# craabreu/EmDee.jl

Hardware: AMD Instinct MI355X
Metric: md_steps_per_sec (higher is better)
Workload: dtype f64

## Files before the change

emdee.jl_amd/csrc/brick.hpp:

```cpp
#pragma once

#include "kernels.hpp"

namespace emdee {

enum BrickMode { BRICK_FORCE = 1, BRICK_STATS = 2, BRICK_STEP = 3 };

#define EMDEE_PLAIN_LOOP _Pragma("clang loop unroll(disable) vectorize(disable) interleave(disable)")

constexpr int EPL = 8;
constexpr int brick_prefetch_blocks(int G, int THREADS) { return (EPL * G) >= 128 ? 1 : ((G == 4 && THREADS >= 1024) ? 5 : 2); }
constexpr int brick_min_stride(int G, int THREADS) { return (brick_prefetch_blocks(G, THREADS) + 1) * EPL * G; }

template <int BX_, int BY_, int BZ_>
struct BrickShape {
    static constexpr int BX = BX_, BY = BY_, BZ = BZ_;
    static constexpr int TX = BX + 2, TY = BY + 2, TZ = BZ + 2;
    static constexpr int NTC = TX * TY * TZ;
    static constexpr int NOC = BX * BY * BZ;
};

struct BrickGrid {
    int nb[3];
    int nbricks;
    int per_xcd;
    int ib_lo[3], ib_n[3];
    int ib_count, ib_per_xcd;
    int bb_z, bb_y, bb_count, bb_per_xcd;
};

__host__ __device__ __forceinline__ int outside_interval(int k, int lo, int n) { return k < lo ? k : k + n; }

template <typename real>
__device__ __forceinline__ void tile_load(const Rec<real> *tile, const float *tile_te, int s, real &x, real &y, real &z,
                                          real &hs, real &te);
template <>
__device__ __forceinline__ void tile_load<double>(const Rec<double> *tile, const float *, int s, double &x, double &y,
                                                  double &z, double &hs, double &te) {
    Rec<double> r = tile[s];
    x = r.x; y = r.y; z = r.z; hs = (double)r.hs; te = (double)r.te;
}
template <>
__device__ __forceinline__ void tile_load<float>(const Rec<float> *tile, const float *tile_te, int s, float &x, float &y,
                                                 float &z, float &hs, float &te) {
    Rec<float> r = tile[s];
// ... 306 lines not shown

template <typename real, class Shape, int THREADS>
__global__ __launch_bounds__(THREADS) void k_brick_tables(BrickArgs<real> a) {
    extern __shared__ __attribute__((aligned(16))) unsigned char s_dyn[];
    BrickTables<Shape, THREADS> T;
    T.carve(s_dyn);
    const int lb = (blockIdx.x % NXCD) * a.bg.per_xcd + blockIdx.x / NXCD;
    if (lb >= a.bg.nbricks) return;
    int bxi = 0, byi = 0, bzi = 0, tile_n = 0, n_own = 0;
    brick_setup<real, Shape, THREADS, true>(a, T, bxi, byi, bzi, tile_n, n_own);
    constexpr int ROW = BrickTables<Shape, THREADS>::row_ints(), IMG = BrickTables<Shape, THREADS>::image_ints();
    int *row = a.btab + (size_t)(bxi + a.bg.nb[0] * (byi + a.bg.nb[1] * bzi)) * ROW;
    for (int i = threadIdx.x; i < IMG; i += THREADS) row[i] = T.off[i];
    if (threadIdx.x == 0) { row[IMG] = tile_n; row[IMG + 1] = n_own; }
    if (a.stats != nullptr) {
        int span3 = 0;
        if (threadIdx.x < Shape::NTC && threadIdx.x % Shape::TX + 3 <= Shape::TX) span3 = T.off[threadIdx.x + 3] - T.off[threadIdx.x];
#pragma unroll
        for (int off = 1; off < WAVE; off <<= 1) span3 = max(span3, __shfl_xor(span3, off));
        int *maxima = reinterpret_cast<int *>(a.stats);
        if ((threadIdx.x & (WAVE - 1)) == 0 && span3 > __hip_atomic_load(&maxima[2], __ATOMIC_RELAXED, __HIP_MEMORY_SCOPE_AGENT)) atomicMax(&maxima[2], span3);
        if (threadIdx.x == 0) {
            if (tile_n - 1 > __hip_atomic_load(&maxima[0], __ATOMIC_RELAXED, __HIP_MEMORY_SCOPE_AGENT)) atomicMax(&maxima[0], tile_n - 1);
            if (n_own > __hip_atomic_load(&maxima[1], __ATOMIC_RELAXED, __HIP_MEMORY_SCOPE_AGENT)) atomicMax(&maxima[1], n_own);
        }
    }
}

constexpr int OWN_REGS = 2;

constexpr int BUILD2_FIELD = 16;

template <typename real, class Shape, int THREADS, int G, int ALG = 1, int GL = G>
__global__ __launch_bounds__(THREADS, (THREADS <= 768 ? 6 : 4)) void k_brick_build(BrickArgs<real> a) {
    constexpr int BX = Shape::BX, BY = Shape::BY, TX = Shape::TX, TY = Shape::TY;
    constexpr int NGROUPS = (THREADS / WAVE) * (WAVE / G);
    extern __shared__ __attribute__((aligned(16))) unsigned char s_dyn[];
    float4 *tile = reinterpret_cast<float4 *>(s_dyn);
    BrickTables<Shape, THREADS> T;
    T.carve(s_dyn + (size_t)a.tile_cap * 16);
    int bxi, byi, bzi, tile_n, n_own;
    if (!brick_setup<real, Shape, THREADS>(a, T, bxi, byi, bzi, tile_n, n_own)) return;
    const int tid = threadIdx.x, lane = tid & (WAVE - 1);
    constexpr bool SUBOK = ALG == 3 || ALG == 5 || ALG == 13 || ALG == 15;
    const int NSUB = (SUBOK && a.nsub == 4 && a.bsub != nullptr) ? 4 : 1;
    unsigned *rtab = reinterpret_cast<unsigned *>(s_dyn + (size_t)a.tile_cap * 16 + BrickTables<Shape, THREADS>::bytes(a.own_cap) +
                                                  (size_t)NGROUPS * a.stride * 2);
    int *s_sub = reinterpret_cast<int *>(s_dyn + (size_t)a.tile_cap * 16 + BrickTables<Shape, THREADS>::bytes(a.own_cap));
    auto rt_get = [](const unsigned *rt, int r) { const unsigned v = rt[r]; return make_int2((int)(v & 0xffffu), (int)(v >> 16)); };
    if (NSUB > 1) {
        const int *bs = a.bsub + (size_t)(bxi + a.bg.nb[0] * (byi + a.bg.nb[1] * bzi)) * Shape::NTC;
        for (int i = tid; i < Shape::NTC; i += THREADS) s_sub[i] = bs[i];
        __syncthreads();
    }
    auto own_sub = [&](int oc, int ti) {
        if (NSUB == 1) return 0;
        const int tc = (oc % BX + 1) + TX * (((oc / BX) % BY + 1) + TY * (oc / (BX * BY) + 1));
        const int kk = ti - T.off[tc], pk = s_sub[tc];
        return (kk >= (pk & 1023) ? 1 : 0) + (kk >= ((pk >> 10) & 1023) ? 1 : 0) + (kk >= ((pk >> 20) & 1023) ? 1 : 0);
    };

    real org[3] = {0, 0, 0};
    if (sizeof(real) == 8) {
        org[0] = a.g.lo[0] + (real)(bxi * BX) * (a.g.len[0] / (real)a.g.M[0]);
        org[1] = a.g.lo[1] + (real)(byi * BY) * (a.g.len[1] / (real)a.g.M[1]);
        org[2] = a.g.lo[2] + (real)(bzi * Shape::BZ) * (a.g.len[2] / (real)a.g.M[2]);
    }
// ... 65 lines not shown
    unsigned short *rowbuf = reinterpret_cast<unsigned short *>(s_dyn + (size_t)a.tile_cap * 16 +
                                                                BrickTables<Shape, THREADS>::bytes(a.own_cap)) +
                             (size_t)gid * a.stride;
    static_assert(G <= 32, "build kernel: groups of at most 32 lanes");
    const unsigned gshift = (unsigned)(lane & 31 & ~(G - 1));
    const unsigned gmask = G == 32 ? 0xffffffffu : ((1u << G) - 1u);
    const unsigned ltmask = (1u << gl) - 1u;
    const bool upper = lane >= 32;
    const unsigned ustride = (unsigned)a.stride;
    const uint4 fill = make_uint4(0, 0, 0, 0);
    auto in_range_q = [&](const float4 &qi, const float4 &qj, int p, int c, int tcr) -> bool {
        const float dx = qi.x - qj.x, dy2 = qi.y - qj.y, dz2 = qi.z - qj.z;
        const float d2 = dx * dx + dy2 * dy2 + dz2 * dz2;
        bool pass = d2 < lo2;
        if (sizeof(real) == 8 && __builtin_expect(!pass && d2 <= hi2, 0)) {
            const int tc = tcr + (c >= T.off[tcr + 1] ? 1 : 0) + (c >= T.off[tcr + 2] ? 1 : 0);
            const int sh = T.shift[tc];
            const Rec<real> ri = a.rec[p], rj = a.rec[__float_as_int(qj.w)];
            const real ex = ri.x - (rj.x + (real)((sh & 3) - 1) * a.g.len[0]);
            const real ey = ri.y - (rj.y + (real)(((sh >> 2) & 3) - 1) * a.g.len[1]);
            const real ez = ri.z - (rj.z + (real)(((sh >> 4) & 3) - 1) * a.g.len[2]);
            pass = ex * ex + ey * ey + ez * ez < a.rlist2;
        }
        return pass;
    };
    auto in_range = [&](const float4 &qi, int p, int c, int tcr) -> bool { return in_range_q(qi, tile[c], p, c, tcr); };
    if constexpr (ALG % 10 == 3 || ALG % 10 == 5) {
        static_assert(G == 4 || G == 8 || G == 16, "two-phase build: 4, 8 or 16 lanes per atom");
        constexpr int FIELD = ALG % 10 == 3 ? BUILD2_FIELD : 32, PER = 32 / FIELD;
        constexpr int NROWS = 9, NWORDS = (NROWS + PER - 1) / PER;
        constexpr bool BAND = sizeof(real) == 8;
        constexpr int UNR = 2;
        float nrl2 = -rl2, nmargin_v = BAND ? -a.margin : 0.f, margin_v = a.margin;
        asm volatile("" : "+v"(nrl2), "+v"(nmargin_v), "+v"(margin_v));
        constexpr bool STRIDED = ALG >= 10;
        constexpr bool OPP = PER == 2;
        auto row_word = [](int r) constexpr { return OPP ? (r <= 4 ? r : 8 - r) : r / PER; };
        auto row_half = [](int r) constexpr { return OPP ? (r > 4 ? 1 : 0) : r % PER; };
        constexpr int LOG2G = G == 4 ? 2 : (G == 8 ? 3 : 4), KSTEP = STRIDED ? G : 1;
        const int wave_first = __builtin_amdgcn_readfirstlane((tid / WAVE) * (WAVE / G));
        for (int ob = 0; ob < n_own; ob += NGROUPS) {
            if (ob + wave_first >= n_own) break;
            const int o = ob + gid;
            const bool have = o < n_own;
            const int2 info = have ? T.oinfo[o] : make_int2(0, 0);
            const int ti = info.y & 0xffff, p = info.x, oc = info.y >> 20;
            const bool act = have && ((info.y >> 16) & 1) != 0;
            const float4 qi = tile[ti];
            unsigned short *row = a.nbr + (size_t)p * a.stride;
            for (int c = gl * EPL; c < a.stride; c += G * EPL) *reinterpret_cast<uint4 *>(rowbuf + c) = fill;
            unsigned word[NWORDS];
            int cbase[NROWS];
            const unsigned *rt = rtab + (act ? oc * NSUB + ((info.y >> 17) & 3) : Shape::NOC * NSUB) * 9;
            int2 rv_next = rt_get(rt, 0);
            int trips_of[NROWS];
            auto chunk_of = [&](int r) { return (int)((unsigned)(rt_get(rt, r).y + G - 1) / (unsigned)G); };
            int cv = chunk_of(min(gl, NROWS - 1));
            int cw = G == 4 ? chunk_of(4 + gl) : 0;
            int c8 = chunk_of(NROWS - 1);
            auto ror4 = [](int v) { return max(v, __builtin_amdgcn_update_dpp(0, v, 0x124 , 0xf, 0xf, true)); };
            auto ror8 = [](int v) { return max(v, __builtin_amdgcn_update_dpp(0, v, 0x128 , 0xf, 0xf, true)); };
            if constexpr (G == 4) { cv = ror4(cv); cw = ror4(cw); c8 = ror4(c8); }
            if constexpr (G <= 8) {
                cv = ror8(cv); c8 = ror8(c8);
                if constexpr (G == 4) cw = ror8(cw);
            }
            auto rows_max = [](int v) {
// ... 92 lines not shown
                    if constexpr (STRIDED) {
                        const int d = ti - c0;
                        if ((d & (G - 1)) == gl) bits &= ~(1u << (d >> LOG2G));
                    } else {
                        const int ks = ti - cb;
                        if (ks >= 0 && ks < lim) bits &= ~(1u << ks);
                    }
                }
                if (row_half(r)) word[row_word(r)] |= bits << (row_half(r) * FIELD);
                else word[row_word(r)] = bits;
            }
            int mine = 0;
#pragma unroll
            for (int w = 0; w < NWORDS; w++) mine += __popc(word[w]);
            int incl = mine;
            {
                int t = __builtin_amdgcn_update_dpp(0, incl, DPP_ROW_SHR1, 0xf, 0xf, true);
                incl += gl >= 1 ? t : 0;
                t = __builtin_amdgcn_update_dpp(0, incl, DPP_ROW_SHR2, 0xf, 0xf, true);
                incl += gl >= 2 ? t : 0;
                if (G >= 8) {
                    t = __builtin_amdgcn_update_dpp(0, incl, DPP_ROW_SHR4, 0xf, 0xf, true);
                    incl += gl >= 4 ? t : 0;
                }
                if (G == 16) {
                    t = __builtin_amdgcn_update_dpp(0, incl, DPP_ROW_SHR8, 0xf, 0xf, true);
                    incl += gl >= 8 ? t : 0;
                }
            }
            unsigned short *ep = rowbuf + (unsigned)(incl - mine), *const ep_last = rowbuf + (ustride - 1u);
#pragma unroll
            for (int w = 0; w < NWORDS; w++) {
                unsigned W = word[w];
                int cA = cbase[OPP ? w : PER * w] << a.idx_shift,
                    cB = (OPP ? (w < 4 ? cbase[8 - w] : 0) : ((PER == 2 && 2 * w + 1 < NROWS) ? cbase[2 * w + 1] : 0)) << a.idx_shift;
                asm volatile("" : "+v"(cA), "+v"(cB));
                const int kshift = a.idx_shift + (STRIDED ? LOG2G : 0);
                while (W) {
                    const int k = __ffs((int)W) - 1;
                    W &= W - 1;
                    asm volatile("" : "+v"(W));
                    *(ep < ep_last ? ep : ep_last) = (unsigned short)((k << kshift) + ((PER == 2 && k >= FIELD) ? cB : cA));
                    ep++;
                }
            }
            if (have && EMDEE_BOUND(BS_BUILD_ROW, p, a.n)) {
                constexpr int BLKL = EPL * GL;
                EMDEE_PLAIN_LOOP
                for (int c = gl * EPL; c < a.stride; c += G * EPL) {
                    const unsigned short *src = rowbuf + (c / BLKL) * BLKL + (c % BLKL) / EPL;
                    uint4 q;
                    q.x = (unsigned)src[0 * GL] | ((unsigned)src[1 * GL] << 16);
                    q.y = (unsigned)src[2 * GL] | ((unsigned)src[3 * GL] << 16);
                    q.z = (unsigned)src[4 * GL] | ((unsigned)src[5 * GL] << 16);
                    q.w = (unsigned)src[6 * GL] | ((unsigned)src[7 * GL] << 16);
                    *reinterpret_cast<uint4 *>(row + c) = q;
                }
                if (gl == G - 1) {
                    a.cnt[p] = act ? (int)min((unsigned)incl, ustride) : 0;
                    if ((unsigned)incl > ustride) atomicMax(&a.flags[0], incl);
                }
            }
        }
        return;
    }
    for (int ob = 0; ob < n_own; ob += NGROUPS) {
        const int o = ob + gid;
        const bool have = o < n_own;
// ... 10 lines not shown
#pragma unroll 1
            for (int dy = -1; dy <= 1; dy++) {
                const int tcr = ox + TX * ((oy + 1 + dy) + TY * (oz + 1 + dz));
                const int c0 = T.off[tcr];
                const int span = act ? T.off[tcr + 3] - c0 : 0;
                const int wspan = wave_group_max<G>(span);
                for (int cb = 0; cb < wspan; cb += G) {
                    const int c = c0 + cb + gl;
                    bool pass = false;
                    if (cb + gl < span && c != ti) pass = in_range(qi, p, c, tcr);
                    const unsigned long long mask = __ballot(pass);
                    const unsigned half = upper ? (unsigned)(mask >> 32) : (unsigned)mask;
                    const unsigned bits = (half >> gshift) & gmask;
                    if (pass) {
                        const unsigned e = count + __popc(bits & ltmask);
                        if (e < ustride && EMDEE_BOUND(BS_BUILD_ROWBUF, row_position<GL>(e), ustride)) rowbuf[row_position<GL>(e)] = (unsigned short)(c << a.idx_shift);
                    }
                    count += __popc(bits);
                }
            }
        }
        if (have && EMDEE_BOUND(BS_BUILD_ROW, p, a.n)) {
            for (int c = gl * EPL; c < a.stride; c += G * EPL)
                *reinterpret_cast<uint4 *>(row + c) = *reinterpret_cast<const uint4 *>(rowbuf + c);
            if (gl == 0) {
                a.cnt[p] = act ? (int)min(count, ustride) : 0;
                if (count > ustride) atomicMax(&a.flags[0], (int)count);
            }
        }
    }
}

template <typename real, class Shape, int THREADS, int G, int MODE, int BITMASK_Q, bool UNI = false>
__global__ __launch_bounds__(THREADS) void k_brick(BrickArgs<real> a) {
    constexpr int BITMASK = BITMASK_Q & ~EMDEE_CHARGED;
    constexpr bool CHG = (BITMASK_Q & EMDEE_CHARGED) != 0;
    static_assert(!CHG || (!UNI && MODE == BRICK_FORCE), "charged instances: general-species force launches only");
    constexpr int NGROUPS = (THREADS / WAVE) * (WAVE / G);
    constexpr int BLK = EPL * G;

    extern __shared__ __attribute__((aligned(16))) unsigned char s_dyn[];
    constexpr bool SOA = UNI && MODE != BRICK_STATS;
    constexpr bool FAST = SOA && BITMASK == EMDEE_FORCES;
    Rec<real> *tile = reinterpret_cast<Rec<real> *>(s_dyn);
    real *plane = reinterpret_cast<real *>(s_dyn);
    constexpr int PITCH = soa_pitch<real>();
    const size_t tile_bytes = SOA ? (((size_t)3 * PITCH * sizeof(real) + 15) & ~(size_t)15) : (size_t)a.tile_cap * sizeof(Rec<real>);
    const size_t te_bytes = (sizeof(real) == 4 && !SOA) ? (((size_t)a.tile_cap * 4 + 15) & ~(size_t)15) : 0;
    float *tile_te = reinterpret_cast<float *>(s_dyn + tile_bytes);
    const size_t q_bytes = CHG ? brick_charge_lds_bytes<real>(a.tile_cap) : 0;
    real *tile_q = reinterpret_cast<real *>(s_dyn + tile_bytes + te_bytes);
    BrickTables<Shape, THREADS> T;
    T.carve(s_dyn + tile_bytes + te_bytes + q_bytes);
    if (MODE == BRICK_STEP && a.guard != nullptr && *a.guard != 0) {
        if (threadIdx.x == 0) *a.trigger = 1;
        return;
    }
    int bxi, byi, bzi, tile_n, n_own;
    if (!brick_setup<real, Shape, THREADS>(a, T, bxi, byi, bzi, tile_n, n_own)) return;
    const int tid = threadIdx.x, lane = tid & (WAVE - 1);
    int own_p[OWN_REGS], own_ti[OWN_REGS], own_m[OWN_REGS];
#pragma unroll
    for (int k = 0; k < OWN_REGS; k++) {
        const int o = tid + k * THREADS;
        own_p[k] = own_ti[k] = own_m[k] = 0;
        if (o < n_own) {
            brick_locate(T, o, own_ti[k], own_p[k]);
// ... 131 lines not shown
                    if (ina | inb) {
                        const f32x2 inv = {fast_rcp(r2.x), fast_rcp(r2.y)};
                        const f32x2 sg2 = {(float)a.uni_sigma2, (float)a.uni_sigma2}, e4v = {(float)a.uni_e4, (float)a.uni_e4};
                        if (BITMASK == EMDEE_FORCES) {
                            f32x2 wr2 = lj_force_over_r2_2(r2, inv, mdl, sg2, e4v);
                            wr2 = f32x2{ina ? wr2.x : 0.f, inb ? wr2.y : 0.f};
                            pfx += wr2 * dx; pfy += wr2 * dy; pfz += wr2 * dz;
                        } else {
                            f32x2 E, W;
                            lj_interaction_pair2(r2, inv, mdl, sg2, e4v, E, W);
                            E = f32x2{ina ? E.x : 0.f, inb ? E.y : 0.f};
                            W = f32x2{ina ? W.x : 0.f, inb ? W.y : 0.f};
                            if (BITMASK & EMDEE_FORCES) {
                                const f32x2 wr2 = W * inv;
                                pfx += wr2 * dx; pfy += wr2 * dy; pfz += wr2 * dz;
                            }
                            if (BITMASK & EMDEE_ENERGIES) pe += E;
                            if (BITMASK & EMDEE_VIRIALS) pw += W;
                            if (BITMASK & EMDEE_TENSOR) {
                                const f32x2 wr2 = W * inv, hx = wr2 * dx, hy = wr2 * dy, hz = wr2 * dz;
                                ptxx += hx * dx; ptyy += hy * dy; ptzz += hz * dz;
                                ptxy += hx * dy; ptxz += hx * dz; ptyz += hy * dz;
                            }
                        }
                    }
                }
            }
        };
        auto block = [&](const uint4 &q, int b0) {
            if constexpr (PACKED) {
                block2(q, b0);
                return;
            }
            constexpr bool AHEAD = SOA && BITMASK == EMDEE_FORCES;
            real xn = 0, yn = 0, zn = 0;
            if (AHEAD) {
                const unsigned char *pn = plane_b + pick16(q, 0);
                xn = *reinterpret_cast<const real *>(pn); yn = *reinterpret_cast<const real *>(pn + PLANE_BYTES);
                zn = *reinterpret_cast<const real *>(pn + 2 * PLANE_BYTES);
            }
#pragma unroll
            for (int t = 0; t < EPL; t++) {
                if (b0 + t * G >= wm) break;
                {
                    const int sj = SOA ? pick16(q, t) : (pick16(q, t) >> a.idx_shift);
                    real xj, yj, zj, hs_j, te_j;
                    if (AHEAD) {
                        xj = xn; yj = yn; zj = zn;
                        if (t + 1 < EPL) {
                            const unsigned char *pj = plane_b + pick16(q, t + 1);
                            xn = *reinterpret_cast<const real *>(pj); yn = *reinterpret_cast<const real *>(pj + PLANE_BYTES);
                            zn = *reinterpret_cast<const real *>(pj + 2 * PLANE_BYTES);
                        }
                        hs_j = te_j = 0;
                    } else if (SOA) {
                        const unsigned char *pj = plane_b + sj;
                        xj = *reinterpret_cast<const real *>(pj);
                        yj = *reinterpret_cast<const real *>(pj + PLANE_BYTES);
                        zj = *reinterpret_cast<const real *>(pj + 2 * PLANE_BYTES);
                        hs_j = te_j = 0;
                    } else tile_load<real>(tile, tile_te, sj, xj, yj, zj, hs_j, te_j);
                    real dx = xi - xj, dy = yi - yj, dz = zi - zj;
                    if (REL && MODE == BRICK_FORCE && !SOA) {
                        if (refmath) {
                            dx = a.g.len[0] * (dx - rint(dx)); dy = a.g.len[1] * (dy - rint(dy)); dz = a.g.len[2] * (dz - rint(dz));
                        }
                    }
                    const real r2 = dx * dx + dy * dy + dz * dz;
                    if (MODE == BRICK_STATS) {
                        st_inside += (b0 + t * G + gl < m && r2 < a.model.rc2) ? 1ull : 0ull;
                    } else if (FAST) {
                        if (r2 < uni.rc2) {
                            const real wr2 = lj_force_over_r2_uni(r2, uni);
                            fx += wr2 * dx; fy += wr2 * dy; fz += wr2 * dz;
                        }
                    } else if (r2 < a.model.rc2) {
                        const real inv_r2 = fast_rcp(r2);
                        if (BITMASK == EMDEE_FORCES) {
                            real wr2;
                            if (UNI) {
                                wr2 = lj_force_over_r2(r2, inv_r2, mdl, a.uni_sigma2, a.uni_e4);
                            } else {
                                const real sg = hs_i + hs_j;
                                wr2 = lj_force_over_r2(r2, inv_r2, mdl, sg * sg, te_i * te_j);
                            }
                            if (CHG) wr2 += rf_force_over_r2(r2, inv_r2, q_i * tile_q[sj], a.chg);
                            fx += wr2 * dx; fy += wr2 * dy; fz += wr2 * dz;
                        } else {
                            real E, W;
                            if (UNI) {
                                lj_interaction_pair(r2, inv_r2, mdl, a.uni_sigma2, a.uni_e4, E, W);
                            } else {
                                lj_interaction(r2, inv_r2, mdl, hs_i, te_i, hs_j, te_j, E, W);
                            }
                            if (CHG) {
                                real Ec, Wc;
                                rf_pair(r2, q_i * tile_q[sj], a.chg, Ec, Wc);
                                E += Ec; W += Wc;
                            }
                            if (BITMASK & EMDEE_FORCES) {
                                const real wr2 = W * inv_r2;
// ... 216 lines not shown
```

emdee.jl_amd/csrc/nbsys.hpp:

```cpp
#pragma once
#include <cstdio>

#include <algorithm>
#include <cmath>
#include <cstdlib>
#include <type_traits>

#include "brick.hpp"
#include "kernels.hpp"
#include "typed.hpp"

namespace emdee {

static inline void refuse_experiment_switches() {
    static const char *const gone[] = {"EMDEE_DEBUG_RC2_SCALE", "EMDEE_TBUILD", "EMDEE_BUILD4", "EMDEE_BUILD_ALG", "EMDEE_BUILD_CHUNKED",
        "EMDEE_BUILD_STRIDED", "EMDEE_NO_BRICK_TABLES", "EMDEE_NO_PREMUL", "EMDEE_BUILD_NEARFAR", "EMDEE_NEAR_DELTA", "EMDEE_FAR_SKIP",
        "EMDEE_PLAN_MAXIMA", "EMDEE_PLAN_SYNC", "EMDEE_STRIDE", "EMDEE_BRICK_VARIANT"};
    for (const char *name : gone)
        EMDEE_REQUIRE(std::getenv(name) == nullptr, EMDEE_ERR_INVALID,
                      "%s is an experiment switch that has been retired with the laboratory (make EXPERIMENTS=1 no longer "
                      "exists): the variant it selected is not built; its measurement is recorded in DESIGN.md, "
                      "\"Product and laboratory\"", name);
}

enum TimerId { T_FORCE = 0, T_KICK_DRIFT = 1, T_REBUILD = 2, T_KICK = 3, T_STEP = 4, T_STEP_BOUNDARY = 5, T_HALO = 6, T_COUNT = 7 };
enum PathId { PATH_BRICK = 0, PATH_DIRECT = 1 };

struct Scanner {
    DevBuf<int> scratch;
    void run(int *data, size_t n, hipStream_t s) {
        if (n == 0) return;
        if (n <= (size_t)SCAN_BLOCK_MAX) {
            hipLaunchKernelGGL(k_scan_block, dim3(1), dim3(1024), 0, s, data, (int)n);
            return;
        }
        size_t total = 0;
        for (size_t m = n; m > 1;) {
            m = (m + SCAN_TILE - 1) / SCAN_TILE;
            total += m;
            if (m == 1) break;
        }
        scratch.ensure(total + 1);
        level(data, n, scratch.ptr, s);
    }

  private:
    void level(int *data, size_t n, int *sums, hipStream_t s) {
        size_t tiles = (n + SCAN_TILE - 1) / SCAN_TILE;
        hipLaunchKernelGGL(k_scan_tiles, dim3((unsigned)tiles), dim3(SCAN_THREADS), 0, s, data, data, n,
                           tiles > 1 ? sums : nullptr);
        if (tiles > 1) {
            level(sums, tiles, sums + tiles, s);
            hipLaunchKernelGGL(k_scan_add, dim3(blocks_for(n, 256)), dim3(256), 0, s, data, n, sums);
        }
    }
};

constexpr size_t LDS_LIMIT = 160 * 1024;

template <int V>
struct BrickVariant;
template <> struct BrickVariant<0> { using Shape = BrickShape<4, 2, 2>; static constexpr int THREADS = 512, G = 4, GB = 8; };
template <> struct BrickVariant<7> { using Shape = BrickShape<4, 2, 2>; static constexpr int THREADS = 1024, G = 4, GB = 8; };
template <> struct BrickVariant<8> { using Shape = BrickShape<4, 2, 2>; static constexpr int THREADS = 1024, G = 8, GB = G; };
template <> struct BrickVariant<9> { using Shape = BrickShape<2, 2, 2>; static constexpr int THREADS = 512, G = 4, GB = 8; };

template <class F>
static inline void with_brick_variant(int v, F &&f) {
    switch (v) {
        case 7: f(BrickVariant<7>{}); break;
        case 8: f(BrickVariant<8>{}); break;
        case 9: f(BrickVariant<9>{}); break;
        default: f(BrickVariant<0>{}); break;
    }
}

template <typename K>
static inline void allow_big_lds(K kernel, size_t bytes) {
    if (bytes > 48 * 1024)
        EMDEE_HIP_CHECK(hipFuncSetAttribute(reinterpret_cast<const void *>(kernel),
                                            hipFuncAttributeMaxDynamicSharedMemorySize, (int)bytes));
}

struct PairTables {
    DevBuf<int> x_start, x_idx;
    DevBuf<int> p_start, p_idx;
    std::vector<int32_t> excl, p14;
    double scale14 = 1.0;
    int rows = 0;
// ... 252 lines not shown
    DevBuf<int> perm, perm2, inv_perm, cell_of, cell_sorted, cell_sorted2, order, count, fill, nbr, cnt, flags, img, img2;
    DevBuf<int2> tmp2;
    DevBuf<long long> tag, tag2;
    bool use_tags = false;
    size_t cap_hint = 0;
    size_t capacity = 0;
    bool has_ghosts = false;
    int id_space = 0;
    bool id_gaps = false;
    DevBuf<int> cmap;
    bool cmap_valid = false;
    SpeciesTable species{1, {0, 0, 0, 0}};
    int nt = 1;
    int nsub = 1;
    bool subbins_enabled = std::getenv("EMDEE_NO_SUBBINS") == nullptr;
    int tsub = 1;
    bool typed_subbins_enabled = std::getenv("EMDEE_TYPED_SUBBINS") == nullptr || std::atoi(std::getenv("EMDEE_TYPED_SUBBINS")) != 0;
    int digits() const { return nt > 1 ? nt * tsub : nsub; }
    DevBuf<int> bsub;
    bool typed_enabled = std::getenv("EMDEE_NO_TYPED") == nullptr;
    DevBuf<int> cstart;
    DevBuf<unsigned long long> species_tab;
    DevBuf<unsigned short> nbr16;
    DevBuf<int> btab;
    bool btab_valid = false;
    DevBuf<double> partial, sums;
    DevBuf<unsigned long long> stats;
    Scanner scanner;

    NbSystem() {
        refuse_experiment_switches();
        if (const char *e = std::getenv("EMDEE_PATH")) path = (std::string(e) == "direct") ? PATH_DIRECT : PATH_BRICK;
        if (const char *e = std::getenv("EMDEE_RUN_AHEAD")) run_ahead = std::max(1, std::min(RUN_AHEAD, std::atoi(e)));
    }

    hipStream_t stream() const { return ctx->stream; }
    AtomView<real> view() const { return AtomView<real>{rec.ptr, te.ptr, rel_grid(rel_now, cell_sorted.ptr)}; }

    bool rel_now = false;
    double rel_lo[3] = {0, 0, 0}, rel_cw[3] = {1, 1, 1};
    int rel_M[3] = {1, 1, 1};
    bool rel_wanted() const {
        return sizeof(real) == 4 && with_vel && !with_mass && !use_tags && !has_ghosts && path == PATH_BRICK &&
               std::getenv("EMDEE_F32_ABS") == nullptr;
    }
    RelGrid rel_grid(bool on, const int *cells) const {
        RelGrid r{};
        for (int d = 0; d < 3; d++) { r.lo[d] = rel_lo[d]; r.cw[d] = rel_cw[d]; r.M[d] = rel_M[d]; }
        r.on = on ? 1 : 0;
        r.cell = cells;
        return r;
    }
    RelGrid rel_grid_next(bool on, const int *cells) const {
        RelGrid r{};
        for (int d = 0; d < 3; d++) { r.lo[d] = (double)grid.lo[d]; r.cw[d] = (double)grid.len[d] / (double)grid.M[d]; r.M[d] = grid.M[d]; }
        r.on = on ? 1 : 0;
        r.cell = cells;
        return r;
    }
    void rel_commit(bool on) {
        rel_now = on;
        for (int d = 0; d < 3; d++) { rel_lo[d] = (double)grid.lo[d]; rel_cw[d] = (double)grid.len[d] / (double)grid.M[d]; rel_M[d] = grid.M[d]; }
    }

    struct Timed {
        NbSystem *s;
// ... 316 lines not shown
            const size_t lds = typed_force_lds_bytes<real, typename V::Shape, V::THREADS>(own_cap);
            allow_big_lds(kernel, lds);
            const int phase = (MODE == BRICK_FORCE || MODE == BRICK_STEP) ? force_phase : 0;
            const int blocks = (phase == 1 ? bgrid.ib_per_xcd : phase == 2 ? bgrid.bb_per_xcd : bgrid.per_xcd) * NXCD;
            if (blocks == 0) return;
            hipLaunchKernelGGL(kernel, dim3(blocks), dim3(V::THREADS), lds, stream(), brick_args(phase));
        }
    }

    template <class V>
    static constexpr bool charged_variant() { return std::is_same<V, BrickVariant<0>>::value || std::is_same<V, BrickVariant<8>>::value; }
    template <class V, int MODE, int BM>
    void launch_brick_kernel() {
        if (typed_active) { launch_typed_kernel<V, MODE, BM>(); return; }
        if constexpr (MODE == BRICK_FORCE && (BM == 1 || BM == 7 || BM == TENSOR_PASS)) {
            if (has_charges()) {
                if constexpr (charged_variant<V>()) launch_brick_kernel_impl<V, MODE, BM | EMDEE_CHARGED, false>();
                else EMDEE_REQUIRE(false, EMDEE_ERR_STATE, "charged engine on brick variant %d", variant);
                return;
            }
        }
        if constexpr (std::is_same<V, BrickVariant<0>>::value && (MODE == BRICK_STEP || (MODE == BRICK_FORCE && (BM == 1 || BM == 7 || BM == TENSOR_PASS)))) {
            if (uniform_atoms && tile_cap <= SOA_SLOTS && idx_shift == PLANE_SHIFT && !(MODE == BRICK_FORCE && sizeof(real) == 4 && refmath && ref_pos != nullptr)) {
                launch_brick_kernel_impl<V, MODE, BM, true>();
                return;
            }
        }
        launch_brick_kernel_impl<V, MODE, BM, false>();
    }

    template <class V, int MODE, int BM, bool UNI>
    void launch_brick_kernel_impl() {
        auto kernel = k_brick<real, typename V::Shape, V::THREADS, V::G, MODE, BM, UNI>;
        const size_t lds = (UNI && MODE != BRICK_STATS) ? brick_force_lds_bytes_soa<real, typename V::Shape, V::THREADS>(own_cap)
                                                        : lds_bytes;
        allow_big_lds(kernel, lds);
        const int phase = (MODE == BRICK_FORCE || MODE == BRICK_STEP) ? force_phase : 0;
        const int blocks = (phase == 1 ? bgrid.ib_per_xcd : phase == 2 ? bgrid.bb_per_xcd : bgrid.per_xcd) * NXCD;
        if (blocks == 0) return;
        hipLaunchKernelGGL(kernel, dim3(blocks), dim3(V::THREADS), lds, stream(), brick_args(phase));
    }

    template <class V>
    void launch_brick_force(int bitmask) {
        if constexpr (std::is_same<V, BrickVariant<0>>::value) {
            switch (bitmask) {
                case 1: launch_brick_kernel<V, BRICK_FORCE, 1>(); return;
                case 2: launch_brick_kernel<V, BRICK_FORCE, 2>(); return;
                case 3: launch_brick_kernel<V, BRICK_FORCE, 3>(); return;
                case 4: launch_brick_kernel<V, BRICK_FORCE, 4>(); return;
                case 5: launch_brick_kernel<V, BRICK_FORCE, 5>(); return;
                case 6: launch_brick_kernel<V, BRICK_FORCE, 6>(); return;
                case TENSOR_PASS: launch_brick_kernel<V, BRICK_FORCE, TENSOR_PASS>(); return;
                default: launch_brick_kernel<V, BRICK_FORCE, 7>(); return;
            }
        }
        if (bitmask == 1) launch_brick_kernel<V, BRICK_FORCE, 1>();
        else if (bitmask == TENSOR_PASS) launch_brick_kernel<V, BRICK_FORCE, TENSOR_PASS>();
        else launch_brick_kernel<V, BRICK_FORCE, 7>();
    }

    void plan_geometry() {
        with_brick_variant(variant, [&](auto v) {
            using V = decltype(v);
            using S = typename V::Shape;
            bgrid.nb[0] = (grid.M[0] + S::BX - 1) / S::BX;
            bgrid.nb[1] = (grid.M[1] + S::BY - 1) / S::BY;
            bgrid.nb[2] = (grid.M[2] + S::BZ - 1) / S::BZ;
            bgrid.nbricks = bgrid.nb[0] * bgrid.nb[1] * bgrid.nb[2];
            bgrid.per_xcd = (bgrid.nbricks + NXCD - 1) / NXCD;
            const int B[3] = {S::BX, S::BY, S::BZ};
            bgrid.ib_count = 1;
            for (int d = 0; d < 3; d++) {
                int lo_b = 0, n_b = bgrid.nb[d];
                if (!grid.per[d]) {
                    lo_b = 1;
                    int hi_b = 1;
                    while (hi_b < bgrid.nb[d] && (hi_b + 1) * B[d] < grid.M[d] - 1) hi_b++;
                    n_b = std::max(0, hi_b - lo_b);
                }
                bgrid.ib_lo[d] = lo_b; bgrid.ib_n[d] = n_b;
                bgrid.ib_count *= n_b;
            }
            bgrid.ib_per_xcd = (bgrid.ib_count + NXCD - 1) / NXCD;
            bgrid.bb_z = (bgrid.nb[2] - bgrid.ib_n[2]) * bgrid.nb[0] * bgrid.nb[1];
            bgrid.bb_y = bgrid.ib_n[2] * (bgrid.nb[1] - bgrid.ib_n[1]) * bgrid.nb[0];
            bgrid.bb_count = bgrid.nbricks - bgrid.ib_count;
            bgrid.bb_per_xcd = (bgrid.bb_count + NXCD - 1) / NXCD;
            row_block = EPL * V::G;
        });
    }
    void launch_tile_max(bool with_build_words = false) {
        with_brick_variant(variant, [&](auto v) {
            using S = typename decltype(v)::Shape;
            if (with_build_words) Zeros().add(flags.ptr, 9).run(stream());
            else Zeros().add(flags.ptr + 6, 3).run(stream());
            hipLaunchKernelGGL((k_brick_tile_max<S>), dim3(blocks_for(bgrid.nbricks, 256)), dim3(256), 0, stream(), bgrid,
                               grid.M[0], grid.M[1], grid.M[2], grid.per[0], grid.per[1], grid.per[2], start(),
                               flags.ptr + 6);
        });
    }
    static int with_headroom(int v) { return (v + v / 32 + 8 + 15) / 16 * 16; }
    bool plan_sizes(int max_tile, int max_own, int max_span3) {
        bool ok = true;
        with_brick_variant(variant, [&](auto v) {
            using V = decltype(v);
            using S = typename V::Shape;
            tile_cap = std::max(64, with_headroom(max_tile + 1));
            if (max_tile + 1 <= SOA_SLOTS) tile_cap = std::min(tile_cap, SOA_SLOTS);
            own_cap = std::max(64, with_headroom(max_own));
            {
                const int exact = std::max(64, (max_tile + 1 + 15) / 16 * 16), st = stride > 0 ? stride : 128;
                constexpr size_t USABLE = 150000;
                auto per_cu = [&](int tc) {
                    const size_t b = brick_build_lds_bytes<S, V::THREADS>(tc, own_cap, st, V::GB, nsub),
                                 f = brick_force_lds_bytes<real, S, V::THREADS>(tc, own_cap, has_charges());
                    return (int)(USABLE / std::max<size_t>(b, 1)) * 16 + (int)(USABLE / std::max<size_t>(f, 1));
                };
                while (tile_cap > exact && per_cu(tile_cap) < per_cu(exact)) tile_cap -= 16;
            }
            plan_span3 = max_span3 + max_span3 / 16 + 2;
            if (std::getenv("EMDEE_DEBUG_PLAN"))
                std::fprintf(stderr, "emdee plan: bricks %d x %d x %d, tile_cap %d (max %d), own_cap %d (max %d), max 3-cell span %d, x sub-bins %d K %d\n", bgrid.nb[0],
                             bgrid.nb[1], bgrid.nb[2], tile_cap, max_tile, own_cap, max_own, max_span3, nsub, sub_k());
            build_alg = (!field16_blocked && (V::GB == 8 || V::GB == 16) && plan_span3 <= BUILD2_FIELD * V::GB) ? 3 : 1;
            if (build_alg == 1 && (V::GB == 8 || V::GB == 16) && plan_span3 <= 32 * V::GB) build_alg = 5;
            if (build_alg == 1) plan_span3 = 1 << 30;
            else plan_span3 = (build_alg == 5 ? 32 : BUILD2_FIELD) * V::GB;
            lds_bytes = brick_force_lds_bytes<real, S, V::THREADS>(tile_cap, own_cap, has_charges());
            ok = lds_bytes <= LDS_LIMIT && tile_cap < 65536;
            build_margin = 0.f;
            if (sizeof(real) == 8) {
                double cmax = 0.0;
                const int B[3] = {S::BX, S::BY, S::BZ};
                for (int d = 0; d < 3; d++) cmax = std::max(cmax, (B[d] + 2) * len[d] / grid.M[d]);
                const double bound = 4.0 * 1.7320508 * rlist * cmax * std::ldexp(1.0, -24) + 4.0 * rlist * rlist * std::ldexp(1.0, -23);
                build_margin = (float)(4.0 * bound);
            }
        });
        return ok;
    }
    int plan_span3 = 0;
    bool plan_holds(const int32_t *maxima) const {
        return maxima[0] + 1 <= tile_cap && maxima[1] <= own_cap && maxima[2] <= plan_span3;
    }
    bool plan_bricks() {
        plan_geometry();
        launch_tile_max();
        read_back_words(ctx, stream(), flags.ptr + 6, 3, ctx->host_flags + 6);
        for (int k = 0; k < 3; k++) plan_maxima[k] = ctx->host_flags[6 + k];
        return plan_sizes(plan_maxima[0], plan_maxima[1], plan_maxima[2]);
    }
    int plan_maxima[3] = {0, 0, 0};

    bool brick_active = false;

    bool build_fits_lds() {
        bool ok = true;
        with_brick_variant(variant, [&](auto v) {
            using V = decltype(v);
            ok = brick_build_lds_bytes<typename V::Shape, V::THREADS>(tile_cap, own_cap, stride, V::GB, nsub) <= LDS_LIMIT;
            if (typed_active) ok = typed_build_lds_bytes<typename V::Shape, V::THREADS>(tile_cap, own_cap, stride, V::GB, V::G) <= LDS_LIMIT;
        });
        return ok;
    }

    bool plan_valid = false;
    int plan_M[3] = {0, 0, 0}, plan_n = 0;
    void make_plan() {
        const int n = n_total;
        variant = 0;
        brick_active = (path == PATH_BRICK) && n > 0 && plan_bricks();
        if (brick_active && lds_bytes > LDS_LIMIT / 2) {
            variant = 8;
            if (!plan_bricks()) { variant = 0; plan_bricks(); }
        }
        if (brick_active) {
            stride = (stride + row_block - 1) / row_block * row_block;
            with_brick_variant(variant, [&](auto v) { stride = std::max(stride, brick_min_stride(decltype(v)::G, decltype(v)::THREADS)); });
        }
        if (brick_active && !build_fits_lds()) brick_active = false;
        idx_shift = (brick_active && variant == 0 && uniform_atoms && !has_charges() && tile_cap <= SOA_SLOTS) ? PLANE_SHIFT : 0;
        typed_active = false;
        if (brick_active && nt == 2 && !typed_blocked && !filters_rows() && !has_charges()) {
            const int keep = variant;
            int cands[2] = {-1, -1};
            if (variant == 8) {
                const char *tb = std::getenv("EMDEE_TYPED_BRICKS");
                const bool only7 = tb != nullptr && std::atoi(tb) == 7;
                cands[0] = only7 ? 7 : 9;
                cands[1] = only7 ? -1 : 7;
            } else if (variant == 7 || variant == 9 || (variant == 0 && std::getenv("EMDEE_TYPED_ALL") != nullptr)) {
                cands[0] = variant;
            }
// ... 114 lines not shown
                            lds_build_bytes = typed_build_lds_bytes<typename V::Shape, V::THREADS>(tile_cap, own_cap, stride, V::GB, V::G);
                            allow_big_lds(kernel, lds_build_bytes);
                            BrickArgs<real> ba = brick_args();
                            ba.nsub = ta.nsub; ba.bsub = ta.bsub;
                            hipLaunchKernelGGL(kernel, dim3(bgrid.per_xcd * NXCD), dim3(V::THREADS), lds_build_bytes, stream(), ba);
                            return;
                        }
                    }
                    if (!btab_valid) {
                        constexpr int TT = V::Shape::NTC <= 128 ? 128 : 256;
                        using BT = BrickTables<typename V::Shape, TT>;
                        static_assert(BT::row_ints() == BrickTables<typename V::Shape, V::THREADS>::row_ints(), "table row layout");
                        btab.ensure((size_t)bgrid.nbricks * BT::row_ints());
                        btab_valid = false;
                        BrickArgs<real> ta = brick_args();
                        ta.btab = btab.ptr;
                        ta.stats = nullptr;
                        if (nsub > 1) { bsub.ensure((size_t)bgrid.nbricks * V::Shape::NTC + 4); ta.bsub = bsub.ptr; }
                        hipLaunchKernelGGL((k_brick_tables<real, typename V::Shape, TT>), dim3(bgrid.per_xcd * NXCD), dim3(TT),
                                           BT::bytes(0), stream(), ta);
                        btab_valid = true;
                    }
                    auto kernel = k_brick_build<real, typename V::Shape, V::THREADS, V::GB, 1, V::G>;
                    if constexpr (V::GB == 8 || V::GB == 16) {
                        if (build_alg == 3) kernel = k_brick_build<real, typename V::Shape, V::THREADS, V::GB, 3, V::G>;
                        if (build_alg == 5) kernel = k_brick_build<real, typename V::Shape, V::THREADS, V::GB, 5, V::G>;
                        if constexpr (V::G == 4) {
                            const bool strided_ok = sizeof(real) == 4 || idx_shift != 0;
                            if (build_alg == 3 && strided_ok) kernel = k_brick_build<real, typename V::Shape, V::THREADS, V::GB, 13, V::G>;
                            if (build_alg == 5 && strided_ok) kernel = k_brick_build<real, typename V::Shape, V::THREADS, V::GB, 15, V::G>;
                        }
                    }
                    lds_build_bytes = brick_build_lds_bytes<typename V::Shape, V::THREADS>(tile_cap, own_cap, stride, V::GB, nsub);
                    allow_big_lds(kernel, lds_build_bytes);
                    hipLaunchKernelGGL(kernel, dim3(bgrid.per_xcd * NXCD), dim3(V::THREADS), lds_build_bytes, stream(),
                                       brick_args());
                });
            } else {
                nbr.ensure(rows * stride);
                if (n > 0)
                    hipLaunchKernelGGL((k_nbr_build<real>), dim3(blocks_for((size_t)n * WAVE, NBR_BLOCK)), dim3(NBR_BLOCK),
                                       0, stream(), n, n_owned, view(), perm.ptr, cell_sorted.ptr, start(), grid,
                                       (real)(rlist * rlist), nbr.ptr, stride, cnt.ptr, flags.ptr);
            }
            if (in_edit && edit_extra.n > 0) {
                read_back_words(ctx, stream(), flags.ptr, 9, ctx->host_flags, edit_extra.dev, edit_extra.n, edit_extra.host);
                edit_extra_read = true;
            } else {
                read_back_words(ctx, stream(), flags.ptr, 9, ctx->host_flags);
            }
            if (kept && (!plan_holds(ctx->host_flags + 6) || ctx->host_flags[2] != 0)) {
                kept = false;
                plan_valid = false;
                btab_valid = false;
                make_plan();
                continue;
            }
            if (brick_active && ctx->host_flags[4] != 0) {
                EMDEE_REQUIRE(!field16_blocked, EMDEE_ERR_OVERFLOW, "neighbour build: a lane's share of a tile row (%d) overflows its hit field", ctx->host_flags[4]);
                field16_blocked = true;
                kept = false; plan_valid = false; btab_valid = false;
                make_plan();
                continue;
            }
            EMDEE_REQUIRE(ctx->host_flags[2] == 0, EMDEE_ERR_OVERFLOW, "LDS tile overflow (%d records > %d)",
                          ctx->host_flags[2], tile_cap);
            int needed = ctx->host_flags[0];
            if (needed <= stride) {
// ... 519 lines not shown
```

Measured before the change: 531.5.

## Add 576-thread brick step and build kernels for dense fp64 single-species boxes

Adds 576-thread instances of the brick force/step and neighbor-build kernels, selected when the mean owned atoms per brick falls between 256 and 288 in uniform fp64 systems. The wider workgroup is meant to cover all owned atoms in one pass rather than leaving a mostly idle second pass. Launch bounds request 7 waves per SIMD, and register pressure is trimmed by dropping the lookahead prefetch, recomputing row bases and using FMA for r2. This risks register spills and adds more template instantiations and selection logic.

Measured after the change: 459.5. -13.6%, worse.

```diff
diff --git a/emdee.jl_amd/csrc/brick.hpp b/emdee.jl_amd/csrc/brick.hpp
--- a/emdee.jl_amd/csrc/brick.hpp
+++ b/emdee.jl_amd/csrc/brick.hpp
@@ -11,6 +11,9 @@
 constexpr int EPL = 8;
 constexpr int brick_prefetch_blocks(int G, int THREADS) { return (EPL * G) >= 128 ? 1 : ((G == 4 && THREADS >= 1024) ? 5 : 2); }
 constexpr int brick_min_stride(int G, int THREADS) { return (brick_prefetch_blocks(G, THREADS) + 1) * EPL * G; }
+constexpr int WIDE_THREADS = 576;
+constexpr int brick_force_min_waves(int THREADS) { return THREADS == WIDE_THREADS ? 7 : 1; }
+constexpr int brick_build_min_waves(int THREADS) { return THREADS == WIDE_THREADS ? 7 : (THREADS <= 768 ? 6 : 4); }
 
 template <int BX_, int BY_, int BZ_>
 struct BrickShape {
@@ -383,7 +386,7 @@
 constexpr int BUILD2_FIELD = 16;
 
 template <typename real, class Shape, int THREADS, int G, int ALG = 1, int GL = G>
-__global__ __launch_bounds__(THREADS, (THREADS <= 768 ? 6 : 4)) void k_brick_build(BrickArgs<real> a) {
+__global__ __launch_bounds__(THREADS, brick_build_min_waves(THREADS)) void k_brick_build(BrickArgs<real> a) {
     constexpr int BX = Shape::BX, BY = Shape::BY, TX = Shape::TX, TY = Shape::TY;
     constexpr int NGROUPS = (THREADS / WAVE) * (WAVE / G);
     extern __shared__ __attribute__((aligned(16))) unsigned char s_dyn[];
@@ -515,7 +518,8 @@
         constexpr bool BAND = sizeof(real) == 8;
         constexpr int UNR = 2;
         float nrl2 = -rl2, nmargin_v = BAND ? -a.margin : 0.f, margin_v = a.margin;
-        asm volatile("" : "+v"(nrl2), "+v"(nmargin_v), "+v"(margin_v));
+        if constexpr (THREADS == WIDE_THREADS) asm volatile("" : "+v"(nrl2), "+v"(margin_v));
+        else asm volatile("" : "+v"(nrl2), "+v"(nmargin_v), "+v"(margin_v));
         constexpr bool STRIDED = ALG >= 10;
         constexpr bool OPP = PER == 2;
         auto row_word = [](int r) constexpr { return OPP ? (r <= 4 ? r : 8 - r) : r / PER; };
@@ -674,8 +678,13 @@
 #pragma unroll
             for (int w = 0; w < NWORDS; w++) {
                 unsigned W = word[w];
-                int cA = cbase[OPP ? w : PER * w] << a.idx_shift,
-                    cB = (OPP ? (w < 4 ? cbase[8 - w] : 0) : ((PER == 2 && 2 * w + 1 < NROWS) ? cbase[2 * w + 1] : 0)) << a.idx_shift;
+                static_assert(THREADS != WIDE_THREADS || STRIDED, "576-thread build: round-robin candidates only");
+                auto base_of = [&](int r) {
+                    if constexpr (THREADS == WIDE_THREADS) return (int)(rt[r] & 0xffffu) + gl - row_half(r) * FIELD * KSTEP;
+                    else return cbase[r];
+                };
+                int cA = base_of(OPP ? w : PER * w) << a.idx_shift,
+                    cB = (OPP ? (w < 4 ? base_of(8 - w) : 0) : ((PER == 2 && 2 * w + 1 < NROWS) ? base_of(2 * w + 1) : 0)) << a.idx_shift;
                 asm volatile("" : "+v"(cA), "+v"(cB));
                 const int kshift = a.idx_shift + (STRIDED ? LOG2G : 0);
                 while (W) {
@@ -752,7 +761,7 @@
 }
 
 template <typename real, class Shape, int THREADS, int G, int MODE, int BITMASK_Q, bool UNI = false>
-__global__ __launch_bounds__(THREADS) void k_brick(BrickArgs<real> a) {
+__global__ __launch_bounds__(THREADS, brick_force_min_waves(THREADS)) void k_brick(BrickArgs<real> a) {
     constexpr int BITMASK = BITMASK_Q & ~EMDEE_CHARGED;
     constexpr bool CHG = (BITMASK_Q & EMDEE_CHARGED) != 0;
     static_assert(!CHG || (!UNI && MODE == BRICK_FORCE), "charged instances: general-species force launches only");
@@ -950,7 +959,7 @@
                 block2(q, b0);
                 return;
             }
-            constexpr bool AHEAD = SOA && BITMASK == EMDEE_FORCES;
+            constexpr bool AHEAD = SOA && BITMASK == EMDEE_FORCES && THREADS != WIDE_THREADS;
             real xn = 0, yn = 0, zn = 0;
             if (AHEAD) {
                 const unsigned char *pn = plane_b + pick16(q, 0);
@@ -984,7 +993,13 @@
                             dx = a.g.len[0] * (dx - rint(dx)); dy = a.g.len[1] * (dy - rint(dy)); dz = a.g.len[2] * (dz - rint(dz));
                         }
                     }
-                    const real r2 = dx * dx + dy * dy + dz * dz;
+                    real r2;
+                    if constexpr (THREADS == WIDE_THREADS) {
+                        static_assert(sizeof(real) == 8 && FAST, "576 threads: the fp64 plane kernels of the MD loop only");
+                        r2 = t == 0 ? __builtin_fma(dz, dz, __builtin_fma(dy, dy, dx * dx)) : __builtin_fma(dz, dz, __builtin_fma(dx, dx, dy * dy));
+                    } else {
+                        r2 = dx * dx + dy * dy + dz * dz;
+                    }
                     if (MODE == BRICK_STATS) {
                         st_inside += (b0 + t * G + gl < m && r2 < a.model.rc2) ? 1ull : 0ull;
                     } else if (FAST) {
diff --git a/emdee.jl_amd/csrc/nbsys.hpp b/emdee.jl_amd/csrc/nbsys.hpp
--- a/emdee.jl_amd/csrc/nbsys.hpp
+++ b/emdee.jl_amd/csrc/nbsys.hpp
@@ -55,6 +55,13 @@
         }
     }
 };
+
+#ifndef EMDEE_WIDE_STEP
+#define EMDEE_WIDE_STEP 1
+#endif
+#ifndef EMDEE_WIDE_BUILD
+#define EMDEE_WIDE_BUILD 1
+#endif
 
 constexpr size_t LDS_LIMIT = 160 * 1024;
 
@@ -373,6 +380,11 @@
         refuse_experiment_switches();
         if (const char *e = std::getenv("EMDEE_PATH")) path = (std::string(e) == "direct") ? PATH_DIRECT : PATH_BRICK;
         if (const char *e = std::getenv("EMDEE_RUN_AHEAD")) run_ahead = std::max(1, std::min(RUN_AHEAD, std::atoi(e)));
+        if (const char *e = std::getenv("EMDEE_BRICK_THREADS")) {
+            forced_threads = std::atoi(e);
+            EMDEE_REQUIRE(forced_threads == 512 || forced_threads == WIDE_THREADS, EMDEE_ERR_INVALID,
+                          "EMDEE_BRICK_THREADS=%s: the brick kernels of the default variant are built for 512 and %d threads", e, WIDE_THREADS);
+        }
     }
 
     hipStream_t stream() const { return ctx->stream; }
@@ -755,13 +767,21 @@
     template <class V, int MODE, int BM, bool UNI>
     void launch_brick_kernel_impl() {
         auto kernel = k_brick<real, typename V::Shape, V::THREADS, V::G, MODE, BM, UNI>;
-        const size_t lds = (UNI && MODE != BRICK_STATS) ? brick_force_lds_bytes_soa<real, typename V::Shape, V::THREADS>(own_cap)
-                                                        : lds_bytes;
+        size_t lds = (UNI && MODE != BRICK_STATS) ? brick_force_lds_bytes_soa<real, typename V::Shape, V::THREADS>(own_cap)
+                                                  : lds_bytes;
+        int threads = V::THREADS;
+        if constexpr (wide_variant<V>() && UNI && BM == 1 && (MODE == BRICK_STEP || MODE == BRICK_FORCE)) {
+            if (wide_step) {
+                kernel = k_brick<real, typename V::Shape, WIDE_THREADS, V::G, MODE, BM, UNI>;
+                lds = brick_force_lds_bytes_soa<real, typename V::Shape, WIDE_THREADS>(own_cap);
+                threads = WIDE_THREADS;
+            }
+        }
         allow_big_lds(kernel, lds);
         const int phase = (MODE == BRICK_FORCE || MODE == BRICK_STEP) ? force_phase : 0;
         const int blocks = (phase == 1 ? bgrid.ib_per_xcd : phase == 2 ? bgrid.bb_per_xcd : bgrid.per_xcd) * NXCD;
         if (blocks == 0) return;
-        hipLaunchKernelGGL(kernel, dim3(blocks), dim3(V::THREADS), lds, stream(), brick_args(phase));
+        hipLaunchKernelGGL(kernel, dim3(blocks), dim3(threads), lds, stream(), brick_args(phase));
     }
 
     template <class V>
@@ -781,6 +801,38 @@
         if (bitmask == 1) launch_brick_kernel<V, BRICK_FORCE, 1>();
         else if (bitmask == TENSOR_PASS) launch_brick_kernel<V, BRICK_FORCE, TENSOR_PASS>();
         else launch_brick_kernel<V, BRICK_FORCE, 7>();
+    }
+
+    int forced_threads = 0;
+    bool wide_step = false, wide_build = false;
+    template <class V>
+    static constexpr bool wide_variant() { return sizeof(real) == 8 && std::is_same<V, BrickVariant<0>>::value; }
+    template <class V>
+    void choose_workgroup() {
+        wide_step = wide_build = false;
+        const bool able = wide_variant<V>() && uniform_atoms && nt == 1 && !has_charges() && tile_cap <= SOA_SLOTS &&
+                          !use_tags && !has_ghosts && cap_hint == 0;
+        const double cells = (double)grid.M[0] * grid.M[1] * grid.M[2];
+        const double mean_own = cells > 0 ? (double)V::Shape::NOC * n_total / cells : 0.0;
+        bool wide = able && mean_own > 256.0 && mean_own + mean_own / 64.0 <= 288.0;
+        if (forced_threads != 0) {
+            EMDEE_REQUIRE(forced_threads != WIDE_THREADS || able, EMDEE_ERR_INVALID,
+                          "EMDEE_BRICK_THREADS=%d: only undivided single-species fp64 boxes on the plane kernels have %d-thread kernels",
+                          WIDE_THREADS, WIDE_THREADS);
+            wide = forced_threads == WIDE_THREADS;
+        }
+        wide_step = wide && WIDE_STEP_DEFAULT_OK;
+        wide_build = wide && WIDE_BUILD_DEFAULT_OK;
+        if ((wide || (forced_threads != 0 && able)) && std::getenv("EMDEE_DEBUG_PLAN"))
+            std::fprintf(stderr, "emdee plan: %.1f own atoms per full brick: step kernels %d threads, build kernel %d threads%s\n", mean_own,
+                         wide_step ? WIDE_THREADS : V::THREADS, wide_build ? WIDE_THREADS : V::THREADS, forced_threads ? " (EMDEE_BRICK_THREADS)" : "");
+    }
+    static constexpr bool WIDE_STEP_DEFAULT_OK = EMDEE_WIDE_STEP != 0, WIDE_BUILD_DEFAULT_OK = EMDEE_WIDE_BUILD != 0;
+    template <class V>
+    size_t build_lds_bytes(int tc, int oc, int st) const {
+        if constexpr (wide_variant<V>())
+            if (wide_build) return brick_build_lds_bytes<typename V::Shape, WIDE_THREADS>(tc, oc, st, V::GB, nsub);
+        return brick_build_lds_bytes<typename V::Shape, V::THREADS>(tc, oc, st, V::GB, nsub);
     }
 
     void plan_geometry() {
@@ -832,11 +884,12 @@
             tile_cap = std::max(64, with_headroom(max_tile + 1));
             if (max_tile + 1 <= SOA_SLOTS) tile_cap = std::min(tile_cap, SOA_SLOTS);
             own_cap = std::max(64, with_headroom(max_own));
+            choose_workgroup<V>();
             {
                 const int exact = std::max(64, (max_tile + 1 + 15) / 16 * 16), st = stride > 0 ? stride : 128;
                 constexpr size_t USABLE = 150000;
                 auto per_cu = [&](int tc) {
-                    const size_t b = brick_build_lds_bytes<S, V::THREADS>(tc, own_cap, st, V::GB, nsub),
+                    const size_t b = build_lds_bytes<V>(tc, own_cap, st),
                                  f = brick_force_lds_bytes<real, S, V::THREADS>(tc, own_cap, has_charges());
                     return (int)(USABLE / std::max<size_t>(b, 1)) * 16 + (int)(USABLE / std::max<size_t>(f, 1));
                 };
@@ -882,7 +935,7 @@
         bool ok = true;
         with_brick_variant(variant, [&](auto v) {
             using V = decltype(v);
-            ok = brick_build_lds_bytes<typename V::Shape, V::THREADS>(tile_cap, own_cap, stride, V::GB, nsub) <= LDS_LIMIT;
+            ok = build_lds_bytes<V>(tile_cap, own_cap, stride) <= LDS_LIMIT;
             if (typed_active) ok = typed_build_lds_bytes<typename V::Shape, V::THREADS>(tile_cap, own_cap, stride, V::GB, V::G) <= LDS_LIMIT;
         });
         return ok;
@@ -1063,8 +1116,16 @@
                         }
                     }
                     lds_build_bytes = brick_build_lds_bytes<typename V::Shape, V::THREADS>(tile_cap, own_cap, stride, V::GB, nsub);
+                    int threads = V::THREADS;
+                    if constexpr (wide_variant<V>()) {
+                        if (wide_build && build_alg == 3 && idx_shift != 0) {
+                            kernel = k_brick_build<real, typename V::Shape, WIDE_THREADS, V::GB, 13, V::G>;
+                            lds_build_bytes = build_lds_bytes<V>(tile_cap, own_cap, stride);
+                            threads = WIDE_THREADS;
+                        }
+                    }
                     allow_big_lds(kernel, lds_build_bytes);
-                    hipLaunchKernelGGL(kernel, dim3(bgrid.per_xcd * NXCD), dim3(V::THREADS), lds_build_bytes, stream(),
+                    hipLaunchKernelGGL(kernel, dim3(bgrid.per_xcd * NXCD), dim3(threads), lds_build_bytes, stream(),
                                        brick_args());
                 });
             } else {
```
